# imgag/ngs-bits

Hardware: AMD Instinct MI355X
Metric: Mreads/sec + achieved HBM GB/s, MappingQC 30x WGS BAM at 1/2/4/8 MI355X (higher is better)
Workload: dtype u8/int32/int64

## Files before the change

ngs-bits_amd/csrc/common.h:

```cpp
#pragma once
#include <hip/hip_runtime.h>
#include <cstdint>
#include <cstdio>
#include <stdexcept>
#include <string>
#include <cctype>
#include <memory>
#include <vector>
#include "../../include/ngsqc.h"
#include "k1_types.h"
#include "cram_plan.h"
#include "switches.h"

namespace ngsqc {

constexpr int K2_REL_STRIDE = 512;
constexpr int K2_MAX_KSH = 3, K2_MIN_KSH = -4;
constexpr int NAME_SHIFT = 12;

void launch_huff_tokens(const uint8_t* d_comp, const BlockDesc* d_blocks, int64_t n_blocks, BlockStatus* d_status,
                        uint32_t* d_pool, uint32_t pool_pages, uint32_t* d_pool_ctr , uint32_t* d_tok_first, uint32_t* d_tok_count,
                        unsigned long long* d_work , const uint32_t* d_order , int max_wgs, int park , hipStream_t s);
void launch_lz77_resolve(const BlockDesc* d_blocks, int64_t n_blocks, uint8_t* d_out, BlockStatus* d_status,
                         const uint32_t* d_pool, const uint32_t* d_tok_first, const uint32_t* d_tok_count, const uint8_t* d_comp, hipStream_t s);
// ... 21 lines not shown

bool is_cram(const uint8_t* d, size_t n);
void cram_set_reference(const char* fasta);
int cram_set_skip_thread(int flags);
void cram_set_skip(int flags);
int cram_skip();
struct CramSelect { struct Region { std::string chr; int32_t start, end; }; std::vector<Region> regions; int64_t max_slices = 0; };
struct ByteImage
{
	std::unique_ptr<uint8_t[]> p; size_t n = 0;
	void make(size_t bytes) { p.reset(new uint8_t[bytes ? bytes : 1]); n = bytes; }
	uint8_t* data() { return p.get(); }
	const uint8_t* data() const { return p.get(); }
	size_t size() const { return n; }
};
int cram_to_bam_image(const uint8_t* d, size_t n, const std::string& path, ByteImage& image, std::string& err, const OpenSwitches& sw, const CramSelect* sel = nullptr, CramQualPlan* defer = nullptr);
double cram_device_quals(const uint8_t* cram_image, const CramQualPlan& plan, uint8_t* d_image, size_t image_bytes, hipStream_t s);

void launch_crc32(const BlockDesc* d_blocks, int64_t n_blocks, const uint8_t* d_out, const uint32_t* d_expected, BlockStatus* d_status, int chains , hipStream_t s);

void launch_index_count(const uint8_t* d_infl, int64_t total, const BlockDesc* d_blocks, int64_t n_entries, int64_t prefix, int ksh, int64_t nm, int64_t from, int32_t* d_start,
                        uint32_t* d_cnt, int64_t* d_next_abs, uint32_t* d_bad, int32_t n_ref, uint16_t* d_rel, hipStream_t s, bool wave_guess = true);
void launch_index_init(const BlockDesc* d_blocks, int64_t n_entries, int64_t prefix, int ksh, int64_t nm, int64_t exp0, bool guess_all, bool assume0 , int32_t* d_start, hipStream_t s);
void launch_index_chain(const BlockDesc* d_blocks, int64_t n_entries, int64_t prefix, int ksh, int64_t nm, int64_t exp0, int64_t total, const int32_t* d_start, const int64_t* d_next, uint32_t* d_viol, long long* d_straddle , hipStream_t s);
void launch_index_write(const uint8_t* d_infl, int64_t total, const BlockDesc* d_blocks, int64_t n_entries, int64_t prefix, int ksh, int64_t nm, const int32_t* d_start,
                        const uint32_t* d_cnt, const int64_t* d_base, const uint16_t* d_rel, int64_t* d_recoff, hipStream_t s);
void launch_scan_counts(const uint32_t* d_cnt, int64_t n, int64_t* d_base, void* d_tmp, hipStream_t s);
void launch_depth_prefix(int32_t* d_diff, int64_t n_slots, void* d_tmp, hipStream_t s);
size_t scan_tmp_bytes(int64_t n);

constexpr int GC_NMAX = 64;
constexpr int LONG_CIGAR = 64;
constexpr int MODE_DEPTH = 3;
constexpr int MODE_COUNT = 4;

enum { A_TOTAL, A_MAPPED, A_ONTARGET, A_NEAR, A_DUP, A_PP, A_INS_CNT, A_SUM_LEN, A_BASES_MAPPED, A_CLIPPED, A_INS_SUM,
       A_USABLE, A_NO_OVERLAP, A_USABLE_RAW, A_USABLE_ROI, A_DP0, A_DP1, A_DP2, A_DP3, A_DP4, A_DD0, A_DD1, A_DD2, A_DD3,
       A_READS_X, A_READS_Y, A_ALG_BYTES, A_COUNT,
       A_MAX_LEN = A_COUNT, A_FIRST_MAX_KEY, A_FIRST_PAIRED, A_LONG_COUNT, A_FIX_TRIM, A_FIX_LEN, A_FIX_CARRY, A_FIX_CNT,
       A_TILE_KEY, A_TILE_PAIRED,
       A_HIST0, A_DEV_TOTAL = A_HIST0 + 1000 };

struct ScanParams
{
	int32_t mode;
	int32_t min_mapq, min_baseq, skip_mismapped;
// ... 96 lines not shown
```

ngs-bits_amd/csrc/handle.h:

```cpp
#pragma once
#include "common.h"
#include <memory>
#include <condition_variable>
#include <mutex>
#include <algorithm>
#include <cstring>
#include <chrono>
#include <atomic>
#include <functional>
#include <thread>
#include <deque>
#include <fstream>
#include <fcntl.h>
#include <sys/mman.h>
#include <sys/stat.h>
#include <unistd.h>

using namespace ngsqc;

namespace ngsqc { namespace lib {
extern thread_local std::string g_open_error;

struct FormatError : std::runtime_error { using std::runtime_error::runtime_error; };
struct ArgError : std::runtime_error { using std::runtime_error::runtime_error; };
// ... 92 lines not shown
		open.clear(); used = 0;
	}
	void discard() { open.clear(); used = 0; (void)hipGetLastError(); }
	~EvLog() { for (hipEvent_t e : pool) (void)hipEventDestroy(e); }
};

inline double wall_ms() { return std::chrono::duration<double, std::milli>(std::chrono::steady_clock::now().time_since_epoch()).count(); }

inline uint16_t rd16(const uint8_t* p) { return (uint16_t)(p[0] | (p[1] << 8)); }
inline uint32_t rd32(const uint8_t* p) { return (uint32_t)p[0] | ((uint32_t)p[1] << 8) | ((uint32_t)p[2] << 16) | ((uint32_t)p[3] << 24); }

constexpr int K1_CHUNK_WAVES_PER_CU = 5;
constexpr int P1_WAVES_PER_CU = 10;
constexpr int N_DEPTH_SETS = 2;

struct DepthSet
{
	std::vector<ngsqc_region> regions; std::vector<int64_t> doff; std::vector<int32_t> rlen; int64_t n_slots = 0; int64_t roi_bases = 0;
	DevBuf<int32_t> d_reg_start, d_reg_end, d_reg_len, d_tid_first, d_tid_last; DevBuf<int64_t> d_doff; DevBuf<int32_t> d_depth; DevBuf<uint8_t> d_tmp;
	bool depth_ready = false;
};

struct TileCtx { const uint8_t* infl; int64_t total; const int64_t* recoff; int64_t n_rec; int64_t ord_base; int tile; bool last; };
}}

using namespace ngsqc::lib;

struct ngsqc_handle
{
	const OpenSwitches osw;
	CallSwitches sw;
	std::string err, path;
	bool from_cram = false;
	bool selection = false;
	int device = 0; int n_cu = 256;
	hipStream_t stream = nullptr;
	hipStream_t s_p1[2] = {nullptr, nullptr};
	hipStream_t s_p2 = nullptr;
	hipStream_t s_crc = nullptr;
	size_t csize = 0;
	std::vector<BlockDesc> blocks; int64_t total = 0;
	std::vector<uint32_t> crc;
	std::vector<uint64_t> member_off;
	DevBuf<uint8_t> d_comp;
	std::vector<std::string> ref_names; std::vector<int64_t> ref_lens; int64_t first_rec = 0; std::string header_text;
	bool planned = false;
	int64_t chunk = 0, nch = 0;
	std::vector<std::pair<int64_t, int64_t>> tiles;
	std::vector<int64_t> tile_first_chunk;
	int64_t pfx = 0, max_tile_bytes = 0, slot_pages = 0;
	DevBuf<BlockDesc> d_kdesc;
	DevBuf<uint32_t> d_tok_first, d_tok_cnt, d_order, d_tok, d_crc, d_pool_ctr; DevBuf<unsigned long long> d_work; DevBuf<BlockStatus> d_status;
	int p1_wgs = 0;
	DevBuf<uint32_t> d_sync_pool; DevBuf<BlockDesc> d_sync_desc; DevBuf<uint32_t> d_sync_u32; DevBuf<BlockStatus> d_sync_st; DevBuf<unsigned long long> d_sync_work;
	static constexpr int MAX_TILE_BUFS = 4;
	int k1_slots = osw.token_slots;
	DevBuf<uint8_t> buf[MAX_TILE_BUFS]; int nbuf = 2;
	int64_t max_tile_members = 0;
	std::vector<hipEvent_t> ev_chunk;
	std::vector<hipEvent_t> ev_tile;
	PinBuf<BlockStatus> p_status; PinBuf<int32_t> p_start; PinBuf<int64_t> p_next; PinBuf<unsigned long long> p_small;
	bool decoded = false; int cur_tile = -1;
	int64_t n_rec = 0; DevBuf<int64_t> d_recoff;
	DevBuf<int64_t> d_long;
	int64_t tile_prefix = 0, tile_total = 0, tile_u_lo = 0, tile_ord_base = 0;
	int64_t carry_len = 0, carry_src = 0, next_ord_base = 0, expected_abs = 0;
	int64_t k1_enq = 0;
	DevBuf<int32_t> d_start; DevBuf<uint32_t> d_cnt; DevBuf<int64_t> d_next, d_base; DevBuf<uint32_t> d_bad; DevBuf<uint8_t> d_scan_tmp; DevBuf<uint16_t> d_rel;
	DepthSet ds[N_DEPTH_SETS]; int cur_ds = 0;
	ngsqc_timings tm{};
	int shard = 0, n_shards = 1;
	int64_t shard_own_members = -1;
	int64_t shard_limit = -1;
	int64_t shard_u_base = 0;
	int64_t shard_first_abs = -1, shard_exit_abs = -1; int shard_last_tile = -1;
	bool verify_crc = osw.verify_crc;
	struct Upload
	{
		std::vector<std::thread> th; std::mutex mu; std::condition_variable cv;
		std::vector<hipEvent_t> ev; std::vector<char> recorded; size_t piece = 0, n_pieces = 0, bytes = 0; std::atomic<size_t> next{0}; std::atomic<bool> cancel{false};
		std::string err; void* map = nullptr; size_t map_n = 0; int fd = -1; double t0 = 0, t_done = 0; size_t done = 0;
		size_t waited[4] = {0, 0, 0, 0};
		struct SPiece { size_t src, dst, bytes; int64_t chunk; };
		std::vector<SPiece> sp; std::vector<size_t> chunk_first;
// ... 53 lines not shown
	ngsqc_handle* h; const bool keep;
	explicit EagerRecoff(ngsqc_handle* hd) : h(hd), keep(hd->lazy_recoff) { h->lazy_recoff = false; }
	~EagerRecoff() { h->lazy_recoff = keep; }
	EagerRecoff(const EagerRecoff&) = delete; EagerRecoff& operator=(const EagerRecoff&) = delete;
};

void walk_bgzf(const uint8_t* file, size_t n, size_t& off, size_t off_end, int64_t max_members, uint64_t& upos, std::vector<BlockDesc>& blocks, std::vector<uint32_t>& crc, std::vector<uint64_t>* file_off = nullptr);
void scan_bgzf(const uint8_t* file, size_t n, std::vector<BlockDesc>& blocks, std::vector<uint32_t>& crc, int64_t& total, std::vector<uint64_t>* file_off, int threads, bool* in_pieces = nullptr);
std::string inflate_error(const ngsqc_handle* h, int64_t member, uint32_t code);
void inflate_sync(ngsqc_handle* h, const std::vector<int64_t>& idx, const std::vector<BlockDesc>& desc, uint8_t* d_out, int level = 0);
void upload_wait(ngsqc_handle* h, size_t end_byte, hipStream_t st, int slot);
void upload_join(ngsqc_handle* h);
void upload_finish(ngsqc_handle* h);
void stream_pass_begin(ngsqc_handle* h);
void stream_pass_end(ngsqc_handle* h);
void stream_wait_chunk(ngsqc_handle* h, int64_t c, hipStream_t st);
void stream_p2_enqueued(ngsqc_handle* h, int64_t c);
void plan_layout(ngsqc_handle* h);
struct RangeRequest { bool by_name = false; uint64_t voff[2] = {0, 0}; const ngsqc_named_region* regions = nullptr; int64_t n_regions = 0; int64_t head_members = 0; };
int open_impl(ngsqc_handle** out, const char* path, const void* bytes, size_t n, int device, int shard = 0, int n_shards = 1, const RangeRequest* range = nullptr);

const int64_t* ensure_recoff(ngsqc_handle* h);
void sync_all(ngsqc_handle* h);
void stream_tiles(ngsqc_handle* h, const std::function<bool(const TileCtx&)>& f);
void for_each_tile(ngsqc_handle* h, const std::function<bool(int)>& f);

constexpr int64_t BGZF_PIECE = 0xff00;
size_t bgzf_max_bytes(int64_t n);
struct BgzfDeflater
{
	DevBuf<uint16_t> prev; DevBuf<uint32_t> tok, sizes; DevBuf<uint64_t> off; DevBuf<uint8_t> slots, scan_tmp;
	int grid = 0; int64_t cap_members = 0;
	void reserve(int64_t max_members, int device);
	size_t run(const uint8_t* d_in, int64_t n, uint8_t* d_out, hipStream_t s, int device, int level = -1);
};

void write_bai(ngsqc_handle* h, const char* out_path, bool csi = false, int min_shift = 14);
}}
```

ngs-bits_amd/csrc/image.hip:

```cpp
#include "handle.h"

namespace ngsqc { namespace lib {
void walk_bgzf(const uint8_t* file, size_t n, size_t& off, size_t off_end, int64_t max_members, uint64_t& upos, std::vector<BlockDesc>& blocks, std::vector<uint32_t>& crc, std::vector<uint64_t>* file_off)
{
	int64_t k = 0;
	while (off < n && off < off_end && k < max_members)
	{
		if (off + 18 > n) throw FormatError("truncated BGZF header");
		const uint8_t* p = file + off;
		if (p[0] != 31 || p[1] != 139 || p[2] != 8 || !(p[3] & 4)) throw FormatError("not a BGZF block (gzip member without BC extra field)");
		uint32_t xlen = rd16(p + 10), bsize = 0; bool found = false;
		size_t x = 12, xend = 12 + (size_t)xlen;
		if (off + xend > n) throw FormatError("truncated BGZF extra field");
		while (x + 4 <= xend) { uint16_t slen = rd16(p + x + 2); if (p[x] == 'B' && p[x + 1] == 'C' && slen == 2) { bsize = rd16(p + x + 4) + 1u; found = true; } x += 4 + slen; }
		if (!found || bsize < xend + 8 || off + bsize > n) throw FormatError("invalid BGZF block size");
		uint32_t isize = rd32(p + bsize - 4);
		if (isize > 65536) throw FormatError("BGZF block inflates to more than 64 KiB");
		if (isize) { blocks.push_back(BlockDesc{(uint64_t)(off + xend), upos, (uint32_t)(bsize - xend - 8), isize}); crc.push_back(rd32(p + bsize - 8)); if (file_off) file_off->push_back((uint64_t)off); }
		upos += isize; off += bsize; ++k;
	}
}
uint32_t bgzf_member_at(const uint8_t* file, size_t n, size_t off)
{
	if (off + 18 > n) return 0;
// ... 502 lines not shown
		ngsqc_handle::Upload* u = h->up; u->sp.clear(); u->chunk_first.assign((size_t)h->nch + 1, 0);
		for (int64_t c = 0; c < h->nch; ++c)
		{
			const int64_t c0 = c * h->chunk, cn = std::min(h->chunk, nb - c0);
			const size_t base = (size_t)(c % h->comp_slots) * h->comp_slot_bytes;
			for (int64_t i = c0; i < c0 + cn; ++i) kd[(size_t)i].cpos = base + (h->blocks[(size_t)i].cpos - h->chunk_lo[(size_t)c]);
			u->chunk_first[(size_t)c] = u->sp.size();
			for (uint64_t o = h->chunk_lo[(size_t)c]; o < chunk_hi[(size_t)c]; o += piece)
				u->sp.push_back(ngsqc_handle::Upload::SPiece{(size_t)o, base + (size_t)(o - h->chunk_lo[(size_t)c]), (size_t)std::min<uint64_t>(piece, chunk_hi[(size_t)c] - o), c});
		}
		u->chunk_first[(size_t)h->nch] = u->sp.size();
	}
	h->d_kdesc.upload(kd, h->stream); h->d_order.upload(ord, h->stream); h->d_crc.upload(h->crc, h->stream);
	h->d_tok_cnt.ensure((size_t)nb + 8); h->d_tok_first.ensure((size_t)nb + 8); h->d_status.ensure((size_t)nb); h->d_work.ensure((size_t)h->nch); h->d_pool_ctr.ensure((size_t)h->nch);
	dbg_stamp(h->osw.debug, "layout: member tables on the device");
	h->d_tok.ensure((size_t)(n_slots * h->slot_pages) * K1_PAGE_WORDS + 16);
	dbg_stamp(h->osw.debug, "layout: token pool allocated");
	for (int i = 0; i < std::min(nt, h->nbuf); ++i) h->buf[i].ensure((size_t)(h->pfx + h->max_tile_bytes) + 64);
	dbg_stamp(h->osw.debug, "layout: tile buffers allocated");
	h->max_tile_members = 0; for (auto& tl : h->tiles) h->max_tile_members = std::max(h->max_tile_members, tl.second);
	h->p_status.ensure((size_t)nb);
	while ((int64_t)h->ev_chunk.size() < 4 * h->nch) { hipEvent_t e; HIPCHK(hipEventCreate(&e)); h->ev_chunk.push_back(e); }
	while ((int)h->ev_tile.size() < 2 * nt) { hipEvent_t e; HIPCHK(hipEventCreateWithFlags(&e, hipEventDisableTiming)); h->ev_tile.push_back(e); }
	h->p_small.ensure(64); h->p_rb.ensure((size_t)ngsqc_handle::RB_TOTAL);
	HIPCHK(hipStreamSynchronize(h->stream));
	h->tm.n_tiles = nt;
	if (h->stream_img && early_pass) { stream_pass_begin(h); h->up->pass_fresh = true; }
	if (h->osw.debug) fprintf(stderr, "[ngsqc] layout: %d tiles, %lld chunks, %d image slots, token pool %.1f GB, tile buffers %.1f GB, %.1f ms\n", nt, (long long)h->nch, h->comp_slots, (double)n_slots * (double)h->slot_pages * K1_PAGE_WORDS * 4e-9, (double)std::min(nt, h->nbuf) * (double)(h->pfx + h->max_tile_bytes) * 1e-9, wall_ms() - pl0);
}

void plan_layout(ngsqc_handle* h)
{
	if (h->plan_thread.joinable())
	{
		h->plan_thread.join();
		if (!h->plan_err.empty()) { const std::string e = h->plan_err; h->plan_err.clear(); throw std::runtime_error(e); }
	}
	plan_layout_now(h);
}


void open_range_common(ngsqc_handle* h, const uint8_t* bytes, size_t n, int device, const RangeRequest& rq)
{
	if (n >= 4 && memcmp(bytes, "CRAM", 4) == 0) throw std::domain_error("a CRAM file has no BGZF members: ngsqc_open / ngsqc_open_memory decode it (cram.hip)");
	init_device(h, device);
	Timer t(h->stream); t.start();
	size_t off = 0; uint64_t upos = 0; std::vector<uint64_t> hdr_off;
// ... 154 lines not shown
```

ngs-bits_amd/csrc/index.hip:

```cpp
#include "common.h"
#include "k2_guess.h"
#include <algorithm>
#include <cstdlib>

namespace ngsqc {

__device__ __forceinline__ bool record_fields_fit(const uint8_t* r, uint32_t bs)
{
	const uint32_t w = ld32u(r + 12), w2 = ld32u(r + 16);
	return record_fields_fit(w & 0xff, w2 & 0xffff, (int32_t)ld32u(r + 20), bs);
}

__global__ __launch_bounds__(256) void index_guess_kernel(const uint8_t* __restrict__ infl, int64_t total, const BlockDesc* __restrict__ blocks, int64_t n_blocks, int64_t prefix, int ksh, int64_t nm, int64_t from,
                                                          int32_t* start, int32_t n_ref)
{
	const int lane = threadIdx.x & 63;
	const int64_t wave = ((int64_t)blockIdx.x * blockDim.x + threadIdx.x) >> 6, n_waves = ((int64_t)gridDim.x * blockDim.x) >> 6;
	for (int64_t b = from + wave; b < n_blocks; b += n_waves)
	{
		if (start[b] != -2) continue;
		int64_t lo, hi; entry_range(blocks, b, prefix, ksh, nm, lo, hi);
		int32_t found = -1;
		for (int64_t base = lo; base < hi && found < 0;)
		{
// ... 90 lines not shown
	while (o < hi)
	{
		if (o + 4 > total) { res = -(o + 10); stop = true; break; }
		uint32_t bs = ld32u(infl + o);
		if (bs < 32) { res = -2; stop = true; break; }
		if (o + 4 + (int64_t)bs > total) { res = -(o + 10); stop = true; break; }
		if (!record_fields_fit(infl + o, bs)) { res = -2; stop = true; break; }
		if (n < stride) rel[b * stride + n] = (uint16_t)(o - lo);
		++n; o += 4 + (int64_t)bs;
	}
	cnt[b] = n; next_abs[b] = stop ? res : o;
	if (stop && res == -2) atomicAdd(bad, 1u);
}

__global__ void index_init_kernel(const BlockDesc* __restrict__ blocks, int64_t n_blocks, int64_t prefix, int ksh, int64_t nm, int64_t exp0, int guess_all, int assume0, int32_t* __restrict__ start)
{
	int64_t b = (int64_t)blockIdx.x * blockDim.x + threadIdx.x;
	if (b >= n_blocks) return;
	int64_t lo, hi; entry_range(blocks, b, prefix, ksh, nm, lo, hi);
	const bool first_piece = b > 0 && (ksh <= 0 || ((b - 1) & ((1ll << ksh) - 1)) == 0);
	start[b] = hi <= lo ? -1 : guess_all ? -2 : (hi <= exp0 ? -1 : (lo <= exp0 ? (int32_t)(exp0 - lo) : (assume0 && first_piece ? 0 : -2)));
}

__global__ void index_chain_kernel(const BlockDesc* __restrict__ blocks, int64_t n_blocks, int64_t prefix, int ksh, int64_t nm, int64_t exp0, int64_t total,
                                   const int32_t* __restrict__ start, const int64_t* __restrict__ next_abs, uint32_t* __restrict__ viol, long long* __restrict__ straddle)
{
	int64_t b = (int64_t)blockIdx.x * blockDim.x + threadIdx.x;
	bool bad = false;
	if (b < n_blocks)
	{
		int64_t lo, hi; entry_range(blocks, b, prefix, ksh, nm, lo, hi);
		const int32_t s = start[b];
		if (hi <= exp0) bad = s != -1;
		else if (lo <= exp0) bad = s != (int32_t)(exp0 - lo);
		if (!bad && s >= 0)
		{
			const int64_t nx = next_abs[b];
			if (nx == -2) bad = false;
			else if (nx == -3) bad = true;
			else if (nx < 0)
			{
				for (int64_t e = b + 1; e < n_blocks && !bad; ++e) bad = start[e] >= 0;
				if (!bad) *straddle = -(nx + 10);
			}
			else
			{
// ... 107 lines not shown
}

void launch_index_guess(const uint8_t* d_infl, int64_t total, const BlockDesc* d_blocks, int64_t n_entries, int64_t prefix, int ksh, int64_t nm, int64_t from, int32_t* d_start, int32_t n_ref, hipStream_t s)
{
	const int64_t n = n_entries - from;
	if (n <= 0) return;
	const int waves = ksh <= -3 ? 8 : ksh < 0 ? 4 : 1;
	if (waves == 4 || waves == 8)
	{
		const dim3 grid((unsigned)(n < 65536 ? n : 65536));
		if (waves == 4) hipLaunchKernelGGL(index_guess_wide_kernel<4>, grid, dim3(256), 0, s, d_infl, total, d_blocks, n_entries, prefix, ksh, nm, from, d_start, n_ref);
		else hipLaunchKernelGGL(index_guess_wide_kernel<8>, grid, dim3(512), 0, s, d_infl, total, d_blocks, n_entries, prefix, ksh, nm, from, d_start, n_ref);
		KCHECK(); return;
	}
	const int64_t wg = (n + 3) / 4;
	hipLaunchKernelGGL(index_guess_kernel, dim3((int)(wg < 256 * 32 ? wg : 256 * 32)), dim3(256), 0, s, d_infl, total, d_blocks, n_entries, prefix, ksh, nm, from, d_start, n_ref); KCHECK();
}

void launch_index_init(const BlockDesc* d_blocks, int64_t n_entries, int64_t prefix, int ksh, int64_t nm, int64_t exp0, bool guess_all, bool assume0, int32_t* d_start, hipStream_t s)
{
	if (n_entries <= 0) return;
	hipLaunchKernelGGL(index_init_kernel, dim3((int)((n_entries + 255) / 256)), dim3(256), 0, s, d_blocks, n_entries, prefix, ksh, nm, exp0, guess_all ? 1 : 0, assume0 ? 1 : 0, d_start); KCHECK();
}
void launch_index_chain(const BlockDesc* d_blocks, int64_t n_entries, int64_t prefix, int ksh, int64_t nm, int64_t exp0, int64_t total, const int32_t* d_start, const int64_t* d_next, uint32_t* d_viol, long long* d_straddle, hipStream_t s)
{
	if (n_entries <= 0) return;
	hipLaunchKernelGGL(index_chain_kernel, dim3((int)((n_entries + 255) / 256)), dim3(256), 0, s, d_blocks, n_entries, prefix, ksh, nm, exp0, total, d_start, d_next, d_viol, d_straddle); KCHECK();
}

void launch_index_write(const uint8_t* d_infl, int64_t total, const BlockDesc* d_blocks, int64_t n_entries, int64_t prefix, int ksh, int64_t nm, const int32_t* d_start,
                        const uint32_t* d_cnt, const int64_t* d_base, const uint16_t* d_rel, int64_t* d_recoff, hipStream_t s)
{
	if (n_entries <= 0) return;
	int grid = (int)((n_entries + 3) / 4);
	hipLaunchKernelGGL(index_write_kernel, dim3(grid), dim3(256), 0, s, d_infl, total, d_blocks, n_entries, prefix, ksh, nm, d_start, d_cnt, d_base, d_rel, d_recoff); KCHECK();
}

void launch_scan_counts(const uint32_t* d_cnt, int64_t n, int64_t* d_base, void* d_tmp, hipStream_t s)
{
	int64_t tiles = (n + SCAN_TILE - 1) / SCAN_TILE;
	int64_t* ts = (int64_t*)d_tmp;
	if (tiles > 0)
	{
		hipLaunchKernelGGL(scan_tile_sums<uint32_t>, dim3((int)tiles), dim3(SCAN_T), 0, s, d_cnt, n, ts); KCHECK();
		hipLaunchKernelGGL(scan_tile_prefix, dim3(1), dim3(SCAN_T), 0, s, ts, tiles); KCHECK();
		hipLaunchKernelGGL((scan_tile_apply<uint32_t, int64_t, false>), dim3((int)tiles), dim3(SCAN_T), 0, s, d_cnt, n, ts, d_base); KCHECK();
// ... 17 lines not shown
```

ngs-bits_amd/csrc/jobs.hip:

```cpp
#include "handle.h"

namespace ngsqc { namespace lib {

void setup_regions(ngsqc_handle* h, DepthSet& D, const ngsqc_region* regions, int64_t n, bool with_depth = true)
{
	const int n_ref = (int)h->ref_names.size();
	D.regions.assign(regions, regions + (n > 0 ? n : 0));
	D.doff.assign((size_t)n + 1, 0); D.rlen.assign((size_t)n, 0);
	std::vector<int32_t> rs((size_t)n), re((size_t)n), tf((size_t)std::max(n_ref, 1), 0), tl((size_t)std::max(n_ref, 1), 0);
	std::vector<uint8_t> seen((size_t)std::max(n_ref, 1), 0);
	int64_t slots = 0, bases = 0;
	for (int64_t i = 0; i < n; ++i)
	{
		const ngsqc_region& r = regions[i];
		if (r.tid < 0 || r.tid >= n_ref) throw ArgError("region with invalid reference id");
		if (r.start < 1 || r.end < r.start) throw ArgError("invalid region range");
		if (i > 0 && regions[i - 1].tid == r.tid) { if (regions[i - 1].end >= r.start) throw ArgError("Merged and sorted BED file required for coverage details statistics!"); }
		else { if (seen[r.tid]) throw ArgError("Merged and sorted BED file required for coverage details statistics!"); seen[r.tid] = 1; tf[r.tid] = (int32_t)i; }
		tl[r.tid] = (int32_t)i + 1;
		rs[i] = r.start; re[i] = r.end; D.rlen[i] = r.end - r.start + 1; D.doff[i] = slots;
		slots += (int64_t)D.rlen[i] + 1; bases += D.rlen[i];
	}
	D.doff[n] = slots; D.n_slots = slots; D.roi_bases = bases;
	D.d_reg_start.upload(rs, h->stream); D.d_reg_end.upload(re, h->stream); D.d_reg_len.upload(D.rlen, h->stream);
// ... 574 lines not shown
	sp.tid_x = -2; sp.tid_y = -2;
	bind_regions(sp, D);
}

struct IndelJob { const ngsqc_indel_window* windows; int64_t n; int32_t include_npp; int64_t* counts; };

void run_job(ngsqc_handle* h, const ngsqc_job_desc* j, ngsqc_job_result* r, ngsqc_shard_summary* shard_out = nullptr, const IndelJob* ij = nullptr)
{
	if (!j || !r) throw ArgError("null argument");
	const bool part = shard_out != nullptr;
	const bool do_map = j->mapping != nullptr, do_depth = j->depth != nullptr, do_sites = j->n_sites > 0, do_reads = j->read_qc != 0;
	const bool do_indel = ij && ij->n > 0;
	if (do_indel && (part || !ij->windows || !ij->counts)) throw ArgError("indel window job without windows / count buffer");
	if (do_map && !part && !r->counters) throw ArgError("mapping job without a counter buffer");
	if (part && (!do_map || do_reads)) throw ArgError("a shard job needs the mapping scan and cannot run the raw-read QC");
	if (do_sites && (!j->sites || !r->site_counts)) throw ArgError("site pileup job without sites / count buffer");
	if (do_reads && !r->read_stats) throw ArgError("raw-read QC job without a result buffer");
	if (j->n_sites < 0) throw ArgError("invalid site count");
	const double w0 = wall_ms();
	dbg_stamp(h->sw.debug, "job: start");
	h->tm.scan_ms = 0; h->tm.scan_kernel_ms = 0; h->tm.scan_launches = 0; h->tm.finalize_ms = 0; h->tm.depth_scan_ms = 0; h->tm.pileup_ms = 0; h->tm.reads_ms = 0; h->tm.scan_algorithmic_bytes = 0;
	Timer total(h->stream); total.start();
	ngsqc_handle::Partial local_map; ScanState dscan; PileupState pile; IndelState indel; ReadsState reads;
	if (part) { delete h->partial; h->partial = new ngsqc_handle::Partial(); }
	ngsqc_handle::Partial& map = part ? *h->partial : local_map;
	if (do_map) { mapping_setup(h, j->mapping, map); map.scan.in_pass_fix = !part; map.scan.begin(h); }
	if (do_depth) { depth_setup(h, j->depth, h->ds[1], dscan); dscan.in_pass_fix = false; dscan.begin(h); }
	if (do_sites) pile.begin(h, j->sites, j->n_sites, j->site_min_mapq, j->site_min_baseq, j->site_include_npp);
	if (do_sites && do_map && !h->sw.no_fused_pileup) pile.attach(map.scan.sp, &map.scan);
	if (do_indel) indel.begin(h, ij->windows, ij->n, ij->include_npp);
	if (do_reads) reads.begin(h, j->read_qc_single_end);
	const double w1 = wall_ms();
	const bool depth_rides = do_depth && (j->depth->min_baseq <= 0 || h->sw.baseq_ride);
	FuseGuard fg(h, do_map ? &map.scan : (depth_rides ? &dscan : nullptr));
	struct LazyGuard { ngsqc_handle* h; ~LazyGuard() { h->lazy_recoff = false; } } lg{h};
	h->lazy_recoff = !part && !do_reads && !do_indel && ((do_map && !do_depth) || (!do_map && depth_rides && !do_sites)) && !h->sw.eager_recoff;
	stream_tiles(h, [&](const TileCtx& c) {
		if (do_map) map.scan.tile(h, c);
		if (part && c.ord_base == 0 && c.n_rec > 0)
		{
			map.head_n = std::min<int64_t>(c.n_rec, ngsqc_handle::Partial::HEAD_MAX);
			map.d_head.ensure((size_t)map.head_n);
			launch_prefix_capture(map.scan.sp, map.head_n, map.d_head.p, h->stream);
		}
		if (do_depth) dscan.tile(h, c);
		if (do_sites) pile.tile(h, c);
// ... 37 lines not shown
	if (do_reads) { reads.end(h, r->read_stats); h->tm.reads_ms = reads.stage_ms; }
	h->cur_ds = do_map || !do_depth ? 0 : 1;
	h->tm.total_ms = total.stop();
	h->tm.job_wall_ms = wall_ms() - w0;
	if (h->sw.debug) fprintf(stderr, "[ngsqc] job: setup %.2f ms, tile stream %.2f ms (K1 %.2f), results %.2f ms\n", w1 - w0, w2 - w1, h->tm.inflate_ms, wall_ms() - w2);
}

DepthSet& cur_depth(ngsqc_handle* h) { return h->ds[h->cur_ds]; }

}}

extern "C" {

void ngsqc_close(ngsqc_handle* h)
{
	if (!h) return;
	struct Hold { Hold() { reaper().hold(); } ~Hold() { reaper().unhold(); } } hold_frees;
	if (h->plan_thread.joinable()) h->plan_thread.join();
	if (h->up) { upload_join(h); delete h->up; h->up = nullptr; }
	if (h->stream) { (void)hipSetDevice(h->device); sync_all(h); }
	for (hipStream_t s : {h->stream, h->s_p1[0], h->s_p1[1], h->s_p2, h->s_crc}) if (s) (void)hipStreamDestroy(s);
	for (hipEvent_t e : h->ev_chunk) (void)hipEventDestroy(e);
	for (hipEvent_t e : h->ev_tile) (void)hipEventDestroy(e);
	delete h->partial;
	delete h;
}

int ngsqc_run_job(ngsqc_handle* h, const ngsqc_job_desc* job, ngsqc_job_result* result) { return guarded(h, [&] { run_job(h, job, result); }); }

int ngsqc_depth_select(ngsqc_handle* h, int32_t which)
{
	return guarded(h, [&] { if (which < 0 || which >= N_DEPTH_SETS) throw ArgError("invalid depth set"); h->cur_ds = which; });
}

int ngsqc_scan_mapping(ngsqc_handle* h, const ngsqc_mapping_params* p, int64_t* counters, double* gc_reads)
{
	return guarded(h, [&] {
		if (!p || !counters) throw ArgError("null argument");
		ngsqc_job_desc j{}; j.mapping = p; ngsqc_job_result r{}; r.counters = counters; r.gc_reads = gc_reads;
		run_job(h, &j, &r);
	});
}

int ngsqc_scan_mapping_partial(ngsqc_handle* h, const ngsqc_mapping_params* p, ngsqc_shard_summary* out)
{
	return guarded(h, [&] {
// ... 354 lines not shown
```

ngs-bits_amd/csrc/tiles.hip:

```cpp
#include "handle.h"

namespace ngsqc { namespace lib {

void enqueue_k1_tile(ngsqc_handle* h, int t)
{
	const int64_t nb = (int64_t)h->blocks.size();
	uint8_t* out_base = h->buf[t % h->nbuf].p + h->pfx;
	const bool k1_serial = h->sw.k1_serial;
	hipStream_t crc_stream = h->s_crc;
	const int64_t cA = h->tile_first_chunk[(size_t)t], cB = h->tile_first_chunk[(size_t)t + 1];
	auto launch_p1 = [&](int64_t c) {
		const int64_t c0 = c * h->chunk, cn = std::min(h->chunk, nb - c0);
		hipEvent_t* e4 = &h->ev_chunk[(size_t)(4 * c)];
		hipStream_t s1 = k1_serial ? h->s_p2 : h->s_p1[c & 1];
		if (c >= h->k1_slots) HIPCHK(hipStreamWaitEvent(s1, h->ev_chunk[(size_t)(4 * (c - h->k1_slots) + 3)], 0));
		if (h->stream_img) stream_wait_chunk(h, c, s1);
		else if (h->up) { const BlockDesc& lb = h->blocks[(size_t)(c0 + cn - 1)]; upload_wait(h, (size_t)(lb.cpos + lb.clen + 64), s1, k1_serial ? 3 : 1 + (int)(c & 1)); }
		HIPCHK(hipEventRecord(e4[0], s1));
		uint32_t* const pool = h->d_tok.p + (size_t)(c % h->k1_slots) * (size_t)h->slot_pages * K1_PAGE_WORDS;
		launch_huff_tokens(h->d_comp.p, h->d_kdesc.p + c0, cn, h->d_status.p + c0, pool, (uint32_t)h->slot_pages, h->d_pool_ctr.p + c, h->d_tok_first.p + c0, h->d_tok_cnt.p + c0, h->d_work.p + c,
		                   h->d_order.p + c0, h->p1_wgs, h->osw.p1_park, s1);
		HIPCHK(hipEventRecord(e4[1], s1));
	};
	auto launch_p2 = [&](int64_t c) {
		const int64_t c0 = c * h->chunk, cn = std::min(h->chunk, nb - c0);
		hipEvent_t* e4 = &h->ev_chunk[(size_t)(4 * c)];
		uint32_t* const pool = h->d_tok.p + (size_t)(c % h->k1_slots) * (size_t)h->slot_pages * K1_PAGE_WORDS;
		HIPCHK(hipStreamWaitEvent(h->s_p2, e4[1], 0));
		if (c == cA && t >= h->nbuf) HIPCHK(hipStreamWaitEvent(h->s_p2, h->ev_tile[(size_t)(2 * (t - h->nbuf) + 1)], 0));
		HIPCHK(hipEventRecord(e4[2], h->s_p2));
		launch_lz77_resolve(h->d_kdesc.p + c0, cn, out_base, h->d_status.p + c0, pool, h->d_tok_first.p + c0, h->d_tok_cnt.p + c0, h->d_comp.p, h->s_p2);
		HIPCHK(hipEventRecord(e4[3], h->s_p2));
		if (h->stream_img) stream_p2_enqueued(h, c);
		if (h->verify_crc)
		{
			if (crc_stream != h->s_p2) HIPCHK(hipStreamWaitEvent(crc_stream, e4[3], 0));
			launch_crc32(h->d_kdesc.p + c0, cn, out_base, h->d_crc.p + c0, h->d_status.p + c0, h->sw.crc_chains, crc_stream);
		}
	};
	for (int64_t c = cA; c < cB; ++c) { launch_p1(c); launch_p2(c); }
	const int64_t f = h->tiles[(size_t)t].first, m = h->tiles[(size_t)t].second;
	hipStream_t s_last = h->verify_crc ? crc_stream : h->s_p2;
	HIPCHK(hipMemcpyAsync(h->p_status.p + f, h->d_status.p + f, (size_t)m * sizeof(BlockStatus), hipMemcpyDeviceToHost, s_last));
	HIPCHK(hipEventRecord(h->ev_tile[(size_t)(2 * t)], s_last));
	h->tm.inflate_launches++;
	h->k1_enq = h->tile_first_chunk[(size_t)t + 1];
}

void finish_k1_tile(ngsqc_handle* h, int t)
{
	HIPCHK(hipEventSynchronize(h->ev_tile[(size_t)(2 * t)]));
	const int64_t f = h->tiles[(size_t)t].first, m = h->tiles[(size_t)t].second;
	std::vector<int64_t> redo;
	for (int64_t i = f; i < f + m; ++i)
	{
		const uint32_t e = h->p_status.p[i].error;
		if (e == K1_ERR_TOKEN_OVERFLOW) redo.push_back(i);
		else if (e) throw FormatError(inflate_error(h, i, e));
	}
	h->tm.members_inflated += m;
	if (redo.empty()) return;
	std::vector<BlockDesc> desc; const uint64_t u_lo = h->blocks[(size_t)f].upos;
	for (int64_t i : redo) { BlockDesc d = h->blocks[(size_t)i]; d.upos -= u_lo; desc.push_back(d); }
	inflate_sync(h, redo, desc, h->buf[t % h->nbuf].p + h->pfx);
}

const int64_t* ensure_recoff(ngsqc_handle* h)
{
	const ngsqc_handle::RecoffArgs& a = h->rw;
	if (h->recoff_tile != a.tile || a.tile < 0)
	{
		h->d_recoff.ensure_slack((size_t)std::max<int64_t>(a.n_rec, 1));
		size_t iv = h->evlog->begin(h->stream, &h->tm.index_ms);
		launch_index_write(a.base, a.total, a.desc, a.ne, a.prefix, a.ksh, a.nm, h->d_start.p, h->d_cnt.p, h->d_base.p, h->d_rel.p, h->d_recoff.p, h->stream);
		h->evlog->end(iv, h->stream);
		h->recoff_tile = a.tile;
	}
	return h->d_recoff.p;
}

void index_tile(ngsqc_handle* h, int t)
{
	const bool dbg = h->sw.debug;
	const int nt = (int)h->tiles.size();
	const bool last = t == nt - 1;
	const int64_t first = h->tiles[(size_t)t].first, nm = h->tiles[(size_t)t].second;
	if (t == 0) { h->carry_len = 0; h->next_ord_base = 0; h->expected_abs = h->first_rec; }
	const int64_t u_lo = (int64_t)h->blocks[(size_t)first].upos;
	const int64_t u_hi = (int64_t)h->blocks[(size_t)(first + nm - 1)].upos + h->blocks[(size_t)(first + nm - 1)].usize;
	const int64_t prefix = h->carry_len;
	const int64_t total = prefix + (u_hi - u_lo);
	const uint8_t* base = h->buf[t % h->nbuf].p + h->pfx - prefix;
	const BlockDesc* d_desc = h->d_kdesc.p + first;
	const bool anchor_by_guess = t == 0 && h->first_rec < 0;
	int64_t exp0 = prefix ? 0 : (h->expected_abs - u_lo);
	if (t == 0)
	{
		h->long_reads = false;
		const int elr = h->sw.long_read_mode;
		if (elr != SW_UNSET) h->long_reads = elr != 0 && !anchor_by_guess;
		else if (!anchor_by_guess && exp0 >= 0 && exp0 + 4 <= total)
		{
			int64_t off = exp0, sum = 0; int n = 0;
			for (; n < 8 && off + 4 <= total; ++n)
			{
				uint32_t bs = 0;
				HIPCHK(hipMemcpyAsync(&bs, base + off, 4, hipMemcpyDeviceToHost, h->stream)); HIPCHK(hipStreamSynchronize(h->stream));
				if (bs < 32 || bs > (1u << 30)) break;
				sum += bs; off += 4 + (int64_t)bs;
			}
			h->long_reads = n > 0 && sum / n > 8192;
		}
		h->lr_failures = 0;
	}
	int ksh = h->sw.walker_shift;
	if (h->long_reads) ksh = h->sw.group_shift == SW_UNSET ? K2_MIN_KSH : -h->sw.group_shift;
	if (anchor_by_guess || (h->k2_plain && !h->long_reads)) ksh = 0;
	const int64_t ne0 = nm + 1;
	int64_t ne = ksh >= 0 ? (nm << ksh) + 1 : ((nm + (1ll << -ksh) - 1) >> -ksh) + 1;
	auto e_lo = [&](int64_t e) -> int64_t { return e == 0 ? 0 : prefix + ((int64_t)h->blocks[(size_t)(first + e - 1)].upos - u_lo); };
	auto e_sz = [&](int64_t e) -> int64_t { return e == 0 ? prefix : (int64_t)h->blocks[(size_t)(first + e - 1)].usize; };
	EvLog& ev = *h->evlog; size_t iv = ev.begin(h->stream, &h->tm.index_ms);
	const size_t ne_max = (size_t)std::max(ne, ne0);
	h->d_start.ensure_slack(ne_max); h->d_cnt.ensure_slack(ne_max + 1); h->d_next.ensure_slack(ne_max + 1); h->d_base.ensure_slack(ne_max + 1); h->d_bad.ensure(4);
	h->d_scan_tmp.ensure_slack(scan_tmp_bytes((int64_t)ne_max) + 64); h->d_rel.ensure_slack((size_t)(ne0 + 1) * K2_REL_STRIDE + 64);
	int64_t from = 0; int rounds = 0; int64_t straddle = -1; bool found_start = !anchor_by_guess; int64_t chain_exit = total;
	const bool tail_may_cut_a_record = h->shard_own_members >= 0 && h->shard + 1 < h->n_shards;
	const bool assume0 = !anchor_by_guess && !h->k2_plain && !h->long_reads;
	launch_index_init(d_desc, ne, prefix, ksh, nm, exp0, anchor_by_guess, assume0, h->d_start.p, h->stream);
	HIPCHK(hipMemsetAsync(h->d_bad.p, 0, 2 * sizeof(uint32_t), h->stream)); HIPCHK(hipMemsetAsync(h->d_bad.p + 2, 0xff, sizeof(long long), h->stream));
	h->fused_tile = -1;
	const bool try_fuse = h->fuse && (h->fuse_ok || h->long_reads) && !anchor_by_guess && (prefix == 0 || h->long_reads) && !h->sw.no_fused_scan;
	const int64_t fuse_limit = h->shard_own_members >= 0 ? prefix + (h->shard_limit - u_lo) : INT64_MAX;
// ... 138 lines not shown
	if (h->carry_len > h->pfx && !last) throw FormatError("a record that straddles two tiles is larger than the carry area (" + std::to_string(h->carry_len) + " > " + std::to_string(h->pfx) + " bytes; raise NGSQC_CARRY_MAX)");
	h->expected_abs = u_lo + (chain_exit - prefix);
	h->next_ord_base = h->tile_ord_base + n_rec;
	h->decoded = true;
}

TileCtx resident_ctx(ngsqc_handle* h)
{
	const int nt = (int)h->tiles.size(); const int t = h->cur_tile;
	return TileCtx{h->buf[t % h->nbuf].p + h->pfx - h->tile_prefix, h->tile_total, h->recoff_tile == t ? h->d_recoff.p : nullptr , h->n_rec, h->tile_ord_base, t, t == nt - 1};
}

void reset_decode_timings(ngsqc_handle* h)
{
	h->tm.inflate_ms = 0; h->tm.index_ms = 0; h->tm.inflate_launches = 0; h->tm.n_records = 0; h->tm.inflate_huff_ms = 0; h->tm.inflate_lz77_ms = 0;
	h->tm.inflate_huff_launches = 0; h->tm.members_inflated = 0; h->tm.tiles_chain_on_device = 0; h->tm.tiles_scan_fused = 0;
}

void sync_all(ngsqc_handle* h)
{
	(void)hipStreamSynchronize(h->s_p1[0]); (void)hipStreamSynchronize(h->s_p1[1]); (void)hipStreamSynchronize(h->s_p2); (void)hipStreamSynchronize(h->s_crc); (void)hipStreamSynchronize(h->stream);
}

void stream_tiles(ngsqc_handle* h, const std::function<bool(const TileCtx&)>& f)
{
	plan_layout(h);
	dbg_stamp(h->sw.debug, "tile stream: layout ready");
	const int nt = (int)h->tiles.size();
	if (nt == 0) { h->decoded = true; h->n_rec = 0; return; }
	if (nt == 1 && h->decoded && h->cur_tile == 0)
	{
		try { if (!h->lazy_recoff) ensure_recoff(h); f(resident_ctx(h)); } catch (...) { h->evlog->discard(); throw; }
		h->evlog->resolve(); return;
	}
	reset_decode_timings(h);
	h->decoded = false; h->cur_tile = -1; h->k1_enq = 0; h->k2_plain = false;
	const bool dbg = h->sw.debug;
	const bool pipelined = h->sw.pipeline;
	HIPCHK(hipMemsetAsync(h->d_work.p, 0, (size_t)h->nch * sizeof(unsigned long long), h->stream));
	HIPCHK(hipMemsetAsync(h->d_pool_ctr.p, 0, (size_t)h->nch * sizeof(uint32_t), h->stream));
	HIPCHK(hipStreamSynchronize(h->stream));
	if (h->stream_img)
	{
		if (!(h->up->pass_running && h->up->pass_fresh)) stream_pass_begin(h);
		h->up->pass_fresh = false;
	}
	try
	{
		const int ahead = pipelined ? h->nbuf - 1 : 0;
		for (int u = 0; u < std::min(nt, std::max(1, ahead)); ++u) enqueue_k1_tile(h, u);
		for (int t = 0; t < nt; ++t)
		{
			const double d0 = wall_ms();
			if (pipelined && t + ahead < nt) enqueue_k1_tile(h, t + ahead);
			const double d1 = wall_ms();
			finish_k1_tile(h, t);
			const double d2 = wall_ms();
			index_tile(h, t);
			const double d3 = wall_ms();
			const bool go_on = f(resident_ctx(h));
			if (dbg) fprintf(stderr, "[ngsqc] tile %d/%d: enqueue next K1 %.2f ms, wait K1 %.2f ms, K2 %.2f ms, consumers %.2f ms (%lld records)\n", t, nt, d1 - d0, d2 - d1, d3 - d2, wall_ms() - d3, (long long)h->n_rec);
			const bool stop = !go_on || t == h->shard_last_tile;
			if (!stop && t + 1 < nt && h->carry_len > 0)
				HIPCHK(hipMemcpyAsync(h->buf[(t + 1) % h->nbuf].p + h->pfx - h->carry_len, h->buf[t % h->nbuf].p + h->pfx - h->tile_prefix + h->carry_src, (size_t)h->carry_len, hipMemcpyDeviceToDevice, h->stream));
			HIPCHK(hipEventRecord(h->ev_tile[(size_t)(2 * t + 1)], h->stream));
			if (stop) { if (t + 1 < nt) { sync_all(h); h->decoded = nt == 1; } break; }
			if (!pipelined && t + 1 < nt) { HIPCHK(hipStreamSynchronize(h->stream)); enqueue_k1_tile(h, t + 1); }
		}
	}
	catch (...) { if (h->stream_img) stream_pass_end(h); sync_all(h); h->evlog->discard(); h->decoded = false; h->cur_tile = -1; throw; }
	h->evlog->resolve();
	if (h->stream_img)
	{
		if (h->k1_enq < h->nch) stream_pass_end(h);
		else { upload_finish(h); stream_pass_end(h); }
	}
	if (h->k1_enq > 0)
	{
		const int64_t c_end = h->k1_enq;
		HIPCHK(hipEventSynchronize(h->ev_chunk[(size_t)(4 * (c_end - 1) + 3)]));
		float ms = 0;
		HIPCHK(hipEventElapsedTime(&ms, h->ev_chunk[0], h->ev_chunk[(size_t)(4 * (c_end - 1) + 3)])); h->tm.inflate_ms = ms;
		for (int64_t c = 0; c < c_end; ++c)
		{
			hipEvent_t* e4 = &h->ev_chunk[(size_t)(4 * c)];
			HIPCHK(hipEventElapsedTime(&ms, e4[0], e4[1])); h->tm.inflate_huff_ms += ms;
			HIPCHK(hipEventElapsedTime(&ms, e4[2], e4[3])); h->tm.inflate_lz77_ms += ms;
		}
		h->tm.inflate_huff_launches = c_end;
	}
	if (nt > 1) { h->decoded = false; }
}

// ... 3 lines not shown
```

Measured before the change: 1178.

## Decouple CRC check from inflate, sample BAM block sizes on device, pre-enqueue K1

Status readback for inflate no longer waits on the CRC stream. CRC results are copied separately and checked after the tile's index and consumer work, so CRC verification overlaps downstream processing. The long-read detection loop, which did up to eight synchronous 4-byte device-to-host copies, becomes a single sampling kernel with one readback. The first K1 tiles are now enqueued by a guard at job start, before mapping setup, so decode overlaps host setup. The cost is more complex error ordering and extra pinned buffers and events.

```diff
diff --git a/ngs-bits_amd/csrc/common.h b/ngs-bits_amd/csrc/common.h
--- a/ngs-bits_amd/csrc/common.h
+++ b/ngs-bits_amd/csrc/common.h
@@ -67,6 +67,7 @@
 void launch_index_count(const uint8_t* d_infl, int64_t total, const BlockDesc* d_blocks, int64_t n_entries, int64_t prefix, int ksh, int64_t nm, int64_t from, int32_t* d_start,
                         uint32_t* d_cnt, int64_t* d_next_abs, uint32_t* d_bad, int32_t n_ref, uint16_t* d_rel, hipStream_t s, bool wave_guess = true);
 void launch_index_init(const BlockDesc* d_blocks, int64_t n_entries, int64_t prefix, int ksh, int64_t nm, int64_t exp0, bool guess_all, bool assume0 , int32_t* d_start, hipStream_t s);
+void launch_index_sample(const uint8_t* d_infl, int64_t total, int64_t exp0, unsigned long long* d_out , hipStream_t s);
 void launch_index_chain(const BlockDesc* d_blocks, int64_t n_entries, int64_t prefix, int ksh, int64_t nm, int64_t exp0, int64_t total, const int32_t* d_start, const int64_t* d_next, uint32_t* d_viol, long long* d_straddle , hipStream_t s);
 void launch_index_write(const uint8_t* d_infl, int64_t total, const BlockDesc* d_blocks, int64_t n_entries, int64_t prefix, int ksh, int64_t nm, const int32_t* d_start,
                         const uint32_t* d_cnt, const int64_t* d_base, const uint16_t* d_rel, int64_t* d_recoff, hipStream_t s);
diff --git a/ngs-bits_amd/csrc/handle.h b/ngs-bits_amd/csrc/handle.h
--- a/ngs-bits_amd/csrc/handle.h
+++ b/ngs-bits_amd/csrc/handle.h
@@ -138,6 +138,7 @@
 };
 
 struct TileCtx { const uint8_t* infl; int64_t total; const int64_t* recoff; int64_t n_rec; int64_t ord_base; int tile; bool last; };
+enum StreamStart { STREAM_NONE, STREAM_EMPTY, STREAM_RESIDENT, STREAM_QUEUED };
 }}
 
 using namespace ngsqc::lib;
@@ -175,7 +176,10 @@
 	int64_t max_tile_members = 0;
 	std::vector<hipEvent_t> ev_chunk;
 	std::vector<hipEvent_t> ev_tile;
-	PinBuf<BlockStatus> p_status; PinBuf<int32_t> p_start; PinBuf<int64_t> p_next; PinBuf<unsigned long long> p_small;
+	std::vector<hipEvent_t> ev_crc;
+	PinBuf<BlockStatus> p_status, p_status_crc; PinBuf<int32_t> p_start; PinBuf<int64_t> p_next; PinBuf<unsigned long long> p_small;
+	DevBuf<unsigned long long> d_kind;
+	StreamStart stream_start = STREAM_NONE;
 	bool decoded = false; int cur_tile = -1;
 	int64_t n_rec = 0; DevBuf<int64_t> d_recoff;
 	DevBuf<int64_t> d_long;
@@ -275,6 +279,15 @@
 
 const int64_t* ensure_recoff(ngsqc_handle* h);
 void sync_all(ngsqc_handle* h);
+void start_tile_stream(ngsqc_handle* h);
+void abort_tile_stream(ngsqc_handle* h);
+struct StreamStartGuard
+{
+	ngsqc_handle* h;
+	explicit StreamStartGuard(ngsqc_handle* hd) : h(hd) { start_tile_stream(h); }
+	~StreamStartGuard() { if (h->stream_start == STREAM_QUEUED) abort_tile_stream(h); h->stream_start = STREAM_NONE; }
+	StreamStartGuard(const StreamStartGuard&) = delete; StreamStartGuard& operator=(const StreamStartGuard&) = delete;
+};
 void stream_tiles(ngsqc_handle* h, const std::function<bool(const TileCtx&)>& f);
 void for_each_tile(ngsqc_handle* h, const std::function<bool(int)>& f);
 
diff --git a/ngs-bits_amd/csrc/image.hip b/ngs-bits_amd/csrc/image.hip
--- a/ngs-bits_amd/csrc/image.hip
+++ b/ngs-bits_amd/csrc/image.hip
@@ -548,7 +548,9 @@
 	h->p_status.ensure((size_t)nb);
 	while ((int64_t)h->ev_chunk.size() < 4 * h->nch) { hipEvent_t e; HIPCHK(hipEventCreate(&e)); h->ev_chunk.push_back(e); }
 	while ((int)h->ev_tile.size() < 2 * nt) { hipEvent_t e; HIPCHK(hipEventCreateWithFlags(&e, hipEventDisableTiming)); h->ev_tile.push_back(e); }
-	h->p_small.ensure(64); h->p_rb.ensure((size_t)ngsqc_handle::RB_TOTAL);
+	h->p_status_crc.ensure((size_t)nb);
+	while ((int)h->ev_crc.size() < nt) { hipEvent_t e; HIPCHK(hipEventCreateWithFlags(&e, hipEventDisableTiming)); h->ev_crc.push_back(e); }
+	h->p_small.ensure(64); h->p_rb.ensure((size_t)ngsqc_handle::RB_TOTAL); h->d_kind.ensure(2);
 	HIPCHK(hipStreamSynchronize(h->stream));
 	h->tm.n_tiles = nt;
 	if (h->stream_img && early_pass) { stream_pass_begin(h); h->up->pass_fresh = true; }
diff --git a/ngs-bits_amd/csrc/index.hip b/ngs-bits_amd/csrc/index.hip
--- a/ngs-bits_amd/csrc/index.hip
+++ b/ngs-bits_amd/csrc/index.hip
@@ -136,6 +136,19 @@
 	start[b] = hi <= lo ? -1 : guess_all ? -2 : (hi <= exp0 ? -1 : (lo <= exp0 ? (int32_t)(exp0 - lo) : (assume0 && first_piece ? 0 : -2)));
 }
 
+__global__ void index_sample_kernel(const uint8_t* __restrict__ infl, int64_t total, int64_t exp0, unsigned long long* __restrict__ out)
+{
+	if (blockIdx.x != 0 || threadIdx.x != 0) return;
+	int64_t off = exp0; unsigned long long n = 0, sum = 0;
+	for (; n < 8 && off + 4 <= total; ++n)
+	{
+		const uint32_t bs = ld32u(infl + off);
+		if (bs < 32 || bs > (1u << 30)) break;
+		sum += bs; off += 4 + (int64_t)bs;
+	}
+	out[0] = n; out[1] = sum;
+}
+
 __global__ void index_chain_kernel(const BlockDesc* __restrict__ blocks, int64_t n_blocks, int64_t prefix, int ksh, int64_t nm, int64_t exp0, int64_t total,
                                    const int32_t* __restrict__ start, const int64_t* __restrict__ next_abs, uint32_t* __restrict__ viol, long long* __restrict__ straddle)
 {
@@ -289,6 +302,11 @@
 	if (n_entries <= 0) return;
 	hipLaunchKernelGGL(index_init_kernel, dim3((int)((n_entries + 255) / 256)), dim3(256), 0, s, d_blocks, n_entries, prefix, ksh, nm, exp0, guess_all ? 1 : 0, assume0 ? 1 : 0, d_start); KCHECK();
 }
+void launch_index_sample(const uint8_t* d_infl, int64_t total, int64_t exp0, unsigned long long* d_out, hipStream_t s)
+{
+	hipLaunchKernelGGL(index_sample_kernel, dim3(1), dim3(64), 0, s, d_infl, total, exp0, d_out); KCHECK();
+}
+
 void launch_index_chain(const BlockDesc* d_blocks, int64_t n_entries, int64_t prefix, int ksh, int64_t nm, int64_t exp0, int64_t total, const int32_t* d_start, const int64_t* d_next, uint32_t* d_viol, long long* d_straddle, hipStream_t s)
 {
 	if (n_entries <= 0) return;
diff --git a/ngs-bits_amd/csrc/jobs.hip b/ngs-bits_amd/csrc/jobs.hip
--- a/ngs-bits_amd/csrc/jobs.hip
+++ b/ngs-bits_amd/csrc/jobs.hip
@@ -620,6 +620,7 @@
 	h->tm.scan_ms = 0; h->tm.scan_kernel_ms = 0; h->tm.scan_launches = 0; h->tm.finalize_ms = 0; h->tm.depth_scan_ms = 0; h->tm.pileup_ms = 0; h->tm.reads_ms = 0; h->tm.scan_algorithmic_bytes = 0;
 	Timer total(h->stream); total.start();
 	ngsqc_handle::Partial local_map; ScanState dscan; PileupState pile; IndelState indel; ReadsState reads;
+	StreamStartGuard k1_ahead(h);
 	if (part) { delete h->partial; h->partial = new ngsqc_handle::Partial(); }
 	ngsqc_handle::Partial& map = part ? *h->partial : local_map;
 	if (do_map) { mapping_setup(h, j->mapping, map); map.scan.in_pass_fix = !part; map.scan.begin(h); }
@@ -703,6 +704,7 @@
 	for (hipStream_t s : {h->stream, h->s_p1[0], h->s_p1[1], h->s_p2, h->s_crc}) if (s) (void)hipStreamDestroy(s);
 	for (hipEvent_t e : h->ev_chunk) (void)hipEventDestroy(e);
 	for (hipEvent_t e : h->ev_tile) (void)hipEventDestroy(e);
+	for (hipEvent_t e : h->ev_crc) (void)hipEventDestroy(e);
 	delete h->partial;
 	delete h;
 }
diff --git a/ngs-bits_amd/csrc/tiles.hip b/ngs-bits_amd/csrc/tiles.hip
--- a/ngs-bits_amd/csrc/tiles.hip
+++ b/ngs-bits_amd/csrc/tiles.hip
@@ -27,7 +27,11 @@
 		hipEvent_t* e4 = &h->ev_chunk[(size_t)(4 * c)];
 		uint32_t* const pool = h->d_tok.p + (size_t)(c % h->k1_slots) * (size_t)h->slot_pages * K1_PAGE_WORDS;
 		HIPCHK(hipStreamWaitEvent(h->s_p2, e4[1], 0));
-		if (c == cA && t >= h->nbuf) HIPCHK(hipStreamWaitEvent(h->s_p2, h->ev_tile[(size_t)(2 * (t - h->nbuf) + 1)], 0));
+		if (c == cA && t >= h->nbuf)
+		{
+			HIPCHK(hipStreamWaitEvent(h->s_p2, h->ev_tile[(size_t)(2 * (t - h->nbuf) + 1)], 0));
+			if (h->verify_crc) HIPCHK(hipStreamWaitEvent(h->s_p2, h->ev_crc[(size_t)(t - h->nbuf)], 0));
+		}
 		HIPCHK(hipEventRecord(e4[2], h->s_p2));
 		launch_lz77_resolve(h->d_kdesc.p + c0, cn, out_base, h->d_status.p + c0, pool, h->d_tok_first.p + c0, h->d_tok_cnt.p + c0, h->d_comp.p, h->s_p2);
 		HIPCHK(hipEventRecord(e4[3], h->s_p2));
@@ -40,11 +44,25 @@
 	};
 	for (int64_t c = cA; c < cB; ++c) { launch_p1(c); launch_p2(c); }
 	const int64_t f = h->tiles[(size_t)t].first, m = h->tiles[(size_t)t].second;
-	hipStream_t s_last = h->verify_crc ? crc_stream : h->s_p2;
-	HIPCHK(hipMemcpyAsync(h->p_status.p + f, h->d_status.p + f, (size_t)m * sizeof(BlockStatus), hipMemcpyDeviceToHost, s_last));
-	HIPCHK(hipEventRecord(h->ev_tile[(size_t)(2 * t)], s_last));
+	HIPCHK(hipMemcpyAsync(h->p_status.p + f, h->d_status.p + f, (size_t)m * sizeof(BlockStatus), hipMemcpyDeviceToHost, h->s_p2));
+	HIPCHK(hipEventRecord(h->ev_tile[(size_t)(2 * t)], h->s_p2));
+	if (h->verify_crc)
+	{
+		HIPCHK(hipMemcpyAsync(h->p_status_crc.p + f, h->d_status.p + f, (size_t)m * sizeof(BlockStatus), hipMemcpyDeviceToHost, crc_stream));
+		HIPCHK(hipEventRecord(h->ev_crc[(size_t)t], crc_stream));
+	}
 	h->tm.inflate_launches++;
 	h->k1_enq = h->tile_first_chunk[(size_t)t + 1];
+}
+
+void finish_crc_tile(ngsqc_handle* h, int t, int64_t upto)
+{
+	if (!h->verify_crc) return;
+	HIPCHK(hipEventSynchronize(h->ev_crc[(size_t)t]));
+	const int64_t f = h->tiles[(size_t)t].first, m = h->tiles[(size_t)t].second;
+	const BlockStatus* st = h->p_status_crc.p;
+	for (int64_t i = f, end = upto < 0 ? f + m : upto; i < end; ++i)
+		if (st[i].error == K1_ERR_CRC) throw FormatError(inflate_error(h, i, K1_ERR_CRC));
 }
 
 void finish_k1_tile(ngsqc_handle* h, int t)
@@ -56,13 +74,17 @@
 	{
 		const uint32_t e = h->p_status.p[i].error;
 		if (e == K1_ERR_TOKEN_OVERFLOW) redo.push_back(i);
-		else if (e) throw FormatError(inflate_error(h, i, e));
+		else if (e && e != K1_ERR_CRC)
+		{
+			finish_crc_tile(h, t, i);
+			throw FormatError(inflate_error(h, i, e));
+		}
 	}
 	h->tm.members_inflated += m;
 	if (redo.empty()) return;
 	std::vector<BlockDesc> desc; const uint64_t u_lo = h->blocks[(size_t)f].upos;
 	for (int64_t i : redo) { BlockDesc d = h->blocks[(size_t)i]; d.upos -= u_lo; desc.push_back(d); }
-	inflate_sync(h, redo, desc, h->buf[t % h->nbuf].p + h->pfx);
+	try { inflate_sync(h, redo, desc, h->buf[t % h->nbuf].p + h->pfx); } catch (...) { finish_crc_tile(h, t, -1); throw; }
 }
 
 const int64_t* ensure_recoff(ngsqc_handle* h)
@@ -101,14 +123,10 @@
 		if (elr != SW_UNSET) h->long_reads = elr != 0 && !anchor_by_guess;
 		else if (!anchor_by_guess && exp0 >= 0 && exp0 + 4 <= total)
 		{
-			int64_t off = exp0, sum = 0; int n = 0;
-			for (; n < 8 && off + 4 <= total; ++n)
-			{
-				uint32_t bs = 0;
-				HIPCHK(hipMemcpyAsync(&bs, base + off, 4, hipMemcpyDeviceToHost, h->stream)); HIPCHK(hipStreamSynchronize(h->stream));
-				if (bs < 32 || bs > (1u << 30)) break;
-				sum += bs; off += 4 + (int64_t)bs;
-			}
+			unsigned long long* ks = h->p_small.p + 48;
+			launch_index_sample(base, total, exp0, h->d_kind.p, h->stream);
+			HIPCHK(hipMemcpyAsync(ks, h->d_kind.p, 2 * sizeof(unsigned long long), hipMemcpyDeviceToHost, h->stream)); HIPCHK(hipStreamSynchronize(h->stream));
+			const int64_t n = (int64_t)ks[0], sum = (int64_t)ks[1];
 			h->long_reads = n > 0 && sum / n > 8192;
 		}
 		h->lr_failures = 0;
@@ -293,21 +311,23 @@
 	(void)hipStreamSynchronize(h->s_p1[0]); (void)hipStreamSynchronize(h->s_p1[1]); (void)hipStreamSynchronize(h->s_p2); (void)hipStreamSynchronize(h->s_crc); (void)hipStreamSynchronize(h->stream);
 }
 
-void stream_tiles(ngsqc_handle* h, const std::function<bool(const TileCtx&)>& f)
-{
+void abort_tile_stream(ngsqc_handle* h)
+{
+	h->stream_start = STREAM_NONE;
+	if (h->stream_img) stream_pass_end(h);
+	sync_all(h); h->evlog->discard(); h->decoded = false; h->cur_tile = -1;
+}
+
+void start_tile_stream(ngsqc_handle* h)
+{
+	h->stream_start = STREAM_NONE;
 	plan_layout(h);
 	dbg_stamp(h->sw.debug, "tile stream: layout ready");
 	const int nt = (int)h->tiles.size();
-	if (nt == 0) { h->decoded = true; h->n_rec = 0; return; }
-	if (nt == 1 && h->decoded && h->cur_tile == 0)
-	{
-		try { if (!h->lazy_recoff) ensure_recoff(h); f(resident_ctx(h)); } catch (...) { h->evlog->discard(); throw; }
-		h->evlog->resolve(); return;
-	}
+	if (nt == 0) { h->stream_start = STREAM_EMPTY; return; }
+	if (nt == 1 && h->decoded && h->cur_tile == 0) { h->stream_start = STREAM_RESIDENT; return; }
 	reset_decode_timings(h);
 	h->decoded = false; h->cur_tile = -1; h->k1_enq = 0; h->k2_plain = false;
-	const bool dbg = h->sw.debug;
-	const bool pipelined = h->sw.pipeline;
 	HIPCHK(hipMemsetAsync(h->d_work.p, 0, (size_t)h->nch * sizeof(unsigned long long), h->stream));
 	HIPCHK(hipMemsetAsync(h->d_pool_ctr.p, 0, (size_t)h->nch * sizeof(uint32_t), h->stream));
 	HIPCHK(hipStreamSynchronize(h->stream));
@@ -318,8 +338,30 @@
 	}
 	try
 	{
+		const int ahead = h->sw.pipeline ? h->nbuf - 1 : 0;
+		for (int u = 0; u < std::min(nt, std::max(1, ahead)); ++u) enqueue_k1_tile(h, u);
+	}
+	catch (...) { abort_tile_stream(h); throw; }
+	h->stream_start = STREAM_QUEUED;
+	dbg_stamp(h->sw.debug, "tile stream: K1 of the first tiles enqueued");
+}
+
+void stream_tiles(ngsqc_handle* h, const std::function<bool(const TileCtx&)>& f)
+{
+	if (h->stream_start == STREAM_NONE) start_tile_stream(h);
+	const StreamStart st = h->stream_start; h->stream_start = STREAM_NONE;
+	const int nt = (int)h->tiles.size();
+	if (st == STREAM_EMPTY) { h->decoded = true; h->n_rec = 0; return; }
+	if (st == STREAM_RESIDENT)
+	{
+		try { if (!h->lazy_recoff) ensure_recoff(h); f(resident_ctx(h)); } catch (...) { h->evlog->discard(); throw; }
+		h->evlog->resolve(); return;
+	}
+	const bool dbg = h->sw.debug;
+	const bool pipelined = h->sw.pipeline;
+	try
+	{
 		const int ahead = pipelined ? h->nbuf - 1 : 0;
-		for (int u = 0; u < std::min(nt, std::max(1, ahead)); ++u) enqueue_k1_tile(h, u);
 		for (int t = 0; t < nt; ++t)
 		{
 			const double d0 = wall_ms();
@@ -327,10 +369,12 @@
 			const double d1 = wall_ms();
 			finish_k1_tile(h, t);
 			const double d2 = wall_ms();
-			index_tile(h, t);
-			const double d3 = wall_ms();
-			const bool go_on = f(resident_ctx(h));
-			if (dbg) fprintf(stderr, "[ngsqc] tile %d/%d: enqueue next K1 %.2f ms, wait K1 %.2f ms, K2 %.2f ms, consumers %.2f ms (%lld records)\n", t, nt, d1 - d0, d2 - d1, d3 - d2, wall_ms() - d3, (long long)h->n_rec);
+			bool go_on = true; double d3 = d2;
+			try { index_tile(h, t); d3 = wall_ms(); go_on = f(resident_ctx(h)); }
+			catch (...) { finish_crc_tile(h, t, -1); throw; }
+			const double d4 = wall_ms();
+			finish_crc_tile(h, t, -1);
+			if (dbg) fprintf(stderr, "[ngsqc] tile %d/%d: enqueue next K1 %.2f ms, wait K1 %.2f ms, K2 %.2f ms, consumers %.2f ms, wait CRC %.2f ms (%lld records)\n", t, nt, d1 - d0, d2 - d1, d3 - d2, d4 - d3, wall_ms() - d4, (long long)h->n_rec);
 			const bool stop = !go_on || t == h->shard_last_tile;
 			if (!stop && t + 1 < nt && h->carry_len > 0)
 				HIPCHK(hipMemcpyAsync(h->buf[(t + 1) % h->nbuf].p + h->pfx - h->carry_len, h->buf[t % h->nbuf].p + h->pfx - h->tile_prefix + h->carry_src, (size_t)h->carry_len, hipMemcpyDeviceToDevice, h->stream));
@@ -339,7 +383,7 @@
 			if (!pipelined && t + 1 < nt) { HIPCHK(hipStreamSynchronize(h->stream)); enqueue_k1_tile(h, t + 1); }
 		}
 	}
-	catch (...) { if (h->stream_img) stream_pass_end(h); sync_all(h); h->evlog->discard(); h->decoded = false; h->cur_tile = -1; throw; }
+	catch (...) { abort_tile_stream(h); throw; }
 	h->evlog->resolve();
 	if (h->stream_img)
 	{
```

Result: faster. 1201 (median of 6 runs) (+1.9%).
